# jnsquire/sregex

Hardware: AMD Instinct MI355X
Metric: GB/s input scanned (whole job), gen-data stream resident in HBM (higher is better)
Workload: dtype u8; 1 GPU; configs[1]: /[a-z]+@[a-z]+\.[a-z]+/ Pike first-match + captures; 1 stream x 4.00 GiB gen-data (abccc.. + 'aaabbccb'); bytes_per_gpu=4294967293, streams_per_gpu=1, segment_bytes=16896, fixup_rounds=0, matches=0, engine=scan, lineage_passes=0, world_size=1

## Files before the change

sregex_amd/csrc/sre_hip_scan.hip:

```cpp
#include <hip/hip_runtime.h>
#include <stdlib.h>
#include "sre_hip_scan.h"
#include "sre_hip_streams.h"
#include "sre_hip_tile.h"

#define SRE_HIP_PIKE_COUNT 2
#define EV_DONE 1
#define EV_POP  2
#define RC_DECLINED (-5)
#define RC_ERROR    (-1)


__global__ void
sre_k_gen_data(uint8_t *__restrict__ dst, uint64_t n, uint64_t body, const uint8_t *__restrict__ tail)
{
    const uint64_t stride = (uint64_t) gridDim.x * blockDim.x * 16;
    for (uint64_t base = ((uint64_t) blockIdx.x * blockDim.x + threadIdx.x) * 16; base < n;
         base += stride)
    {
        uint8_t  v[16];
        unsigned ph = (unsigned) (base % 5);
#pragma unroll
        for (int k = 0; k < 16; k++) {
            uint64_t i = base + k;
// ... 130 lines not shown
{
    if (c == '\n') return 1u;
    if (T.word_restart && ((c - '0') < 10u || ((c | 32u) - 'a') < 26u || c == '_')) return 3u;
    return 2u;
}

__device__ inline uint32_t
restart_variant(const sre_scan_tables_t &T, const uint8_t *data, int64_t sp)
{
    return restart_variant_of(T, data[sp - 1]);
}

enum : uint32_t {
    F_HAS_EV = 1u, F_LM_VALID = 2u, F_FINISHED = 4u, F_ERROR = 8u, F_UNRESOLVED = 16u, F_SKIP_NEXT = 32u,
    F_IN_PENDING = 64u, F_SP_DIRTY = 128u,
    F_SHADOW = 256u,
    F_PEND_LAZY = 512u,
    F_NO_EOF = 2048u,
    F_LZ_GROUP = 1024u
};

struct Walk {
    const sre_scan_tables_t *T;
    const uint8_t           *data;
    const uint16_t          *tr2;
    int64_t                  n;
    uint32_t st;
    uint32_t fl;
    __device__ inline bool f(uint32_t b) const { return (fl & b) != 0; }
    __device__ inline void set(uint32_t b, bool v) { fl = v ? (fl | b) : (fl & ~b); }
    uint8_t  ev_kind;
    uint32_t ev_state, ev_sym;
    int64_t  ev_pos, ev_sp;
    int64_t  ev_apos;
    uint32_t ev_astate;
    int64_t  cur_sp;
    int64_t  warm_lo;
    int64_t  anchor_pos;
    uint32_t anchor_state;
    uint32_t lm_state, lm_sym;
    int64_t  lm_pos, lm_sp, lm_apos;
    uint32_t lm_astate;
    int64_t  count;
    int64_t  term_pos;

    __device__ void complete_match()
    {
        count++;
        fl |= F_LM_VALID;
        lm_state = ev_state;
        lm_sym = ev_sym;
        lm_pos = ev_pos;
        lm_sp = ev_sp;
        lm_apos = ev_apos;
        lm_astate = ev_astate;
        fl &= ~F_HAS_EV;
    }
};

template <int MODE>
__device__ void slow_run(Walk &w, int64_t p, int64_t p_to, bool warm, uint32_t warm_seed)
{
    const sre_scan_tables_t &T = *w.T;
    const uint32_t           nsym = T.ncls + 1;
    int64_t  win_at = -1;
    uint64_t win_bytes = 0;
    auto byte_at = [&](int64_t q) -> uint32_t {
        const int64_t a = q & ~(int64_t) 7;
        if (a != win_at) {
            win_at = a;
            if (a + 8 <= w.n && ((reinterpret_cast<uintptr_t>(w.data) + (uint64_t) a) & 7u) == 0) {
                win_bytes = *reinterpret_cast<const uint64_t *>(w.data + a);
            } else {
                win_bytes = 0;
                for (int64_t k = 0; k < 8 && a + k < w.n; k++) win_bytes |= (uint64_t) w.data[a + k] << (8 * k);
            }
        }
        return (uint32_t) (win_bytes >> (8 * (q & 7))) & 0xffu;
    };

    if (MODE == SRE_HIP_PIKE_COUNT && w.f(F_SKIP_NEXT)) {
        w.fl &= ~F_SKIP_NEXT;
        p++;
    }
    while (p < p_to && !w.f(F_FINISHED)) {
        if (p == w.n && ((T.state_flags[w.st] >> 1) & 3) == 2) {
            w.term_pos = p;
            if (MODE == SRE_HIP_PIKE_COUNT) {
                if (w.f(F_HAS_EV)) {
                    w.complete_match();
                    w.fl |= F_ERROR;
                }
            } else if (w.f(F_HAS_EV) || (T.state_flags[w.st] & 1)) {
                w.fl |= F_ERROR;
            }
            w.fl |= F_FINISHED;
            return;
        }
        const uint32_t         sym = p < w.n ? T.cls[byte_at(p)] : T.ncls;
        const uint32_t tr2 = w.tr2[w.st * nsym + sym];
        struct { uint32_t next; uint8_t kind; } tr = {tr2 & 0xffu, (uint8_t) (tr2 >> 8)};
        if (tr.kind) {
            w.fl |= F_HAS_EV;
            w.ev_kind = tr.kind;
            w.ev_state = w.st;
            w.ev_sym = sym;
            w.ev_pos = p;
            w.ev_sp = w.cur_sp;
            if (w.anchor_pos >= 0 && w.anchor_pos <= p && p - w.anchor_pos <= 256
                && (w.cur_sp < 0 || w.anchor_pos > w.cur_sp))
            {
                w.ev_apos = w.anchor_pos;
                w.ev_astate = w.anchor_state;
            } else {
                w.ev_apos = -1;
                w.ev_astate = 0;
            }
            if (MODE != SRE_HIP_PIKE_COUNT && !warm) {
                w.fl |= F_LM_VALID;
                w.lm_state = w.st;
                w.lm_sym = sym;
                w.lm_pos = p;
                w.lm_sp = w.cur_sp;
                w.lm_apos = w.ev_apos;
                w.lm_astate = w.ev_astate;
            }
        }
        w.st = (tr.kind && T.mode == 0 && !warm) ? 0u : tr.next;
        if (w.st != 0) {
            p++;
            continue;
        }

        if (warm) {
            if (MODE == SRE_HIP_PIKE_COUNT) {
                if (w.f(F_HAS_EV)) {
                    const bool    pop = (w.ev_kind == EV_POP || w.ev_kind == SRE_DEV_EV_POP_FULL);
                    const bool    empty = w.ev_kind == EV_POP || w.ev_kind == SRE_DEV_EV_DONE_EMPTY;
                    const int64_t e = pop ? w.ev_pos : w.ev_pos + 1;
                    const int64_t sp = empty ? e + 1 : e;
                    if (e >= w.warm_lo && sp >= 1 && !(empty && e >= w.n)) {
                        w.fl &= ~F_HAS_EV;
                        w.cur_sp = sp;
                        w.st = T.init[restart_variant_of(T, byte_at(sp - 1))];
                        p = sp;
                        if (p > p_to && p_to <= w.n) w.fl |= F_SKIP_NEXT;
                        continue;
                    }
                }
                w.st = p < w.n ? T.init[restart_variant_of(T, byte_at(p))] : warm_seed;
            } else {
                w.st = warm_seed;
            }
            w.fl &= ~F_HAS_EV;
            w.cur_sp = -1;
            p++;
            continue;
        }
        if (MODE != SRE_HIP_PIKE_COUNT) {
            w.term_pos = p;
            w.fl |= F_FINISHED;
            return;
        }
        if (!w.f(F_HAS_EV)) {
            if (p < w.n) w.fl |= F_UNRESOLVED;
            w.term_pos = p;
            w.fl |= F_FINISHED;
            return;
        }
        {
            const bool    pop = (w.ev_kind == EV_POP || w.ev_kind == SRE_DEV_EV_POP_FULL);
            const bool    empty = w.ev_kind == EV_POP || w.ev_kind == SRE_DEV_EV_DONE_EMPTY;
            const int64_t e = pop ? w.ev_pos : w.ev_pos + 1;
            w.complete_match();
            if (empty) {
                if (e >= w.n) {
                    w.term_pos = p;
                    w.fl |= F_FINISHED;
                    return;
                }
                w.cur_sp = e + 1;
            } else {
                w.cur_sp = e;
            }
            w.st = T.init[restart_variant_of(T, byte_at(w.cur_sp - 1))];
            p = w.cur_sp;
            if (p > p_to && p_to <= w.n) w.fl |= F_SKIP_NEXT;
            w.anchor_pos = -1;
        }
    }
}

struct SpanResult {
    int64_t  sp;
    int64_t  last_pos, last_sp;
    uint32_t last_state, last_sym;
    int64_t  pend_pos;
    uint32_t pend_state, pend_sym;
};

__device__ __attribute__((noinline)) SpanResult
resolve_fast_span(const sre_scan_tables_t *Tp, const uint16_t *tr2, const uint8_t *data, int64_t gpos,
                  uint32_t len, uint32_t s0, int64_t sp0, int64_t pend0_pos, uint32_t pend0_state, uint32_t pend0_sym)
{
    const sre_scan_tables_t &T = *Tp;
    SpanResult r;
    uint32_t   st = s0;
    r.sp = sp0;
    r.last_pos = r.last_sp = -1;
    r.last_state = r.last_sym = 0;
    r.pend_pos = pend0_pos;
    r.pend_state = pend0_state;
    r.pend_sym = pend0_sym;
    for (uint32_t b = 0; b < len; b++) {
        const uint32_t         sym = T.cls[data[gpos + b]];
        const uint32_t t2 = tr2[st * (T.ncls + 1) + sym];
        struct { uint32_t next; uint8_t kind; } tr = {t2 & 0xffu, (uint8_t) (t2 >> 8)};
        if (tr.kind && tr.next == 0) {
            const bool pop = tr.kind == SRE_DEV_EV_POP_FULL && gpos + b > 0;
            r.last_pos = gpos + b;
            r.last_state = st;
            r.last_sym = sym;
            r.last_sp = r.sp;
            r.sp = pop ? gpos + b : gpos + b + 1;
            r.pend_pos = -1;
            st = T.init[restart_variant(T, data, r.sp)];
            if (pop) st = tr2[st * (T.ncls + 1) + sym] & 0xffu;
        } else if (tr.kind) {
            r.pend_pos = gpos + b;
            r.pend_state = st;
            r.pend_sym = sym;
            st = tr.next;
        } else if (tr.next == 0 && gpos + b > 0) {
            r.last_pos = r.pend_pos;
            r.last_state = r.pend_state;
            r.last_sym = r.pend_sym;
            r.last_sp = r.sp;
            r.sp = gpos + b;
            st = T.init[restart_variant(T, data, r.sp)];
            const uint32_t t3 = tr2[st * (T.ncls + 1) + sym];
            r.pend_pos = -1;
            if ((t3 >> 8) && (t3 & 0xffu) == 0) {
                r.last_pos = gpos + b;
                r.last_state = st;
                r.last_sym = sym;
                r.last_sp = r.sp;
                r.sp = gpos + b + 1;
                st = T.init[restart_variant(T, data, r.sp)];
            } else {
                if (t3 >> 8) {
                    r.pend_pos = gpos + b;
                    r.pend_state = st;
                    r.pend_sym = sym;
                }
                st = t3 & 0xffu;
            }
        } else {
            st = tr.next;
        }
    }
    return r;
}

template <int H>
__device__ inline uint32_t
add_w0_w(uint32_t a, uint32_t b)
{
    uint32_t r;
    if (H == 0) asm("v_add_u32_sdwa %0, %1, %2 dst_sel:DWORD dst_unused:UNUSED_PAD src0_sel:WORD_0 src1_sel:WORD_0" : "=v"(r) : "v"(a), "v"(b));
    if (H == 1) asm("v_add_u32_sdwa %0, %1, %2 dst_sel:DWORD dst_unused:UNUSED_PAD src0_sel:WORD_0 src1_sel:WORD_1" : "=v"(r) : "v"(a), "v"(b));
    if (H == 2) asm("v_add_u32_sdwa %0, %1, %2 dst_sel:DWORD dst_unused:UNUSED_PAD src0_sel:WORD_0 src1_sel:DWORD" : "=v"(r) : "v"(a), "v"(b));
    return r;
}

__device__ inline uint32_t
add_b3(uint32_t a, uint32_t b)
{
    uint32_t r;
    asm("v_add_u32_sdwa %0, %1, %2 dst_sel:DWORD dst_unused:UNUSED_PAD src0_sel:DWORD src1_sel:BYTE_3" : "=v"(r) : "v"(a), "v"(b));
    return r;
}

template <int K>
__device__ inline uint32_t
byte_x4(uint32_t v, uint32_t sh)
{
    uint32_t r;
    if (K == 0) asm("v_lshlrev_b32_sdwa %0, %1, %2 dst_sel:DWORD dst_unused:UNUSED_PAD src0_sel:DWORD src1_sel:BYTE_0" : "=v"(r) : "v"(sh), "v"(v));
    if (K == 1) asm("v_lshlrev_b32_sdwa %0, %1, %2 dst_sel:DWORD dst_unused:UNUSED_PAD src0_sel:DWORD src1_sel:BYTE_1" : "=v"(r) : "v"(sh), "v"(v));
    if (K == 2) asm("v_lshlrev_b32_sdwa %0, %1, %2 dst_sel:DWORD dst_unused:UNUSED_PAD src0_sel:DWORD src1_sel:BYTE_2" : "=v"(r) : "v"(sh), "v"(v));
    if (K == 3) asm("v_lshlrev_b32_sdwa %0, %1, %2 dst_sel:DWORD dst_unused:UNUSED_PAD src0_sel:DWORD src1_sel:BYTE_3" : "=v"(r) : "v"(sh), "v"(v));
    return r;
}

#ifdef SRE_NO_TAIL_PRIO
#define SRE_TAIL_PRIO() ((void) 0)
#else
#define SRE_TAIL_PRIO() __builtin_amdgcn_s_setprio(3)
#endif

#ifndef SRE_SCAN_PREFETCH
#define SRE_SCAN_PREFETCH 1
#endif
#ifndef SRE_FIRST_BLOCKS
#define SRE_FIRST_BLOCKS 4
#endif
#ifndef SRE_COUNT_BLOCKS
#define SRE_COUNT_BLOCKS 3
#endif

template <int MODE, int BITS, bool WIDE, bool GROW>
__global__ __launch_bounds__(SRE_SCAN_BLOCK, MODE == SRE_HIP_PIKE_COUNT ? SRE_COUNT_BLOCKS : SRE_FIRST_BLOCKS) void
sre_k_scan(const sre_scan_tables_t *__restrict__ tabp, sre_scan_geom_t G,
           sre_seg_summary_t *__restrict__ sum, const sre_stream_status_t *__restrict__ st_lo,
           const uint8_t *__restrict__ entry)
{
    constexpr int      TILE = SRE_SCAN_ROUND;
    constexpr int      WARM = SRE_SCAN_LINE;
    constexpr int      STRIDE = 8 / BITS;
    constexpr uint32_t ROWRAW = TILE / STRIDE * (WIDE ? 2 : 1);
    constexpr uint32_t ROWB = 2 * ROWRAW + 16;
    constexpr int      GIDX = 16 / STRIDE;
    typedef const __attribute__((address_space(3))) uint32_t *lds_u32_t;
    extern __shared__ __attribute__((aligned(16))) uint8_t lds[];
    __shared__ uint16_t clsx[BITS == 8 ? 1 : 8 / BITS][256];
    __shared__ sre_scan_tables_t Ts;

    const uint32_t tid = threadIdx.x;
    const uint32_t nst = tabp->nstates, nrows = tabp->fast_rows, nsh = tabp->nshadow;
    uint32_t *fast = reinterpret_cast<uint32_t *>(lds);
    uint8_t  *clsl = lds + nrows * SRE_FAST_ROW_BYTES;
    uint8_t  *trl = clsl + 256;
    const uint32_t tr_bytes = (nst * (tabp->ncls + 1) * 2u + 15u) & ~15u;
    uint8_t  *sfl = trl + tr_bytes;
    uint8_t  *tile = lds + (((size_t) (sfl - lds) + nst + 15u) & ~(size_t) 15u);
    RowDesc  *rows = reinterpret_cast<RowDesc *>(tile + SRE_SCAN_BLOCK * ROWB);
    (void) nrows;
    if (tid == 0) {
        Ts = *tabp;
        Ts.cls = clsl;
        Ts.state_flags = sfl;
    }
    constexpr uint32_t LDS_SLOW = 1u << 16;
    constexpr uint32_t LDS_CNT_SHIFT = 24;
    constexpr uint32_t LDS_FRESH = 1u << 17;
    const uint32_t fast_lds = (uint32_t) (uintptr_t) (__attribute__((address_space(3))) uint8_t *) lds;
    const uint32_t trap_lds = fast_lds + nst * SRE_FAST_ROW_BYTES;
    const uint32_t shadow_lds = trap_lds + SRE_FAST_ROW_BYTES;
    auto to_lds = [fast_lds, trap_lds](uint32_t g) -> uint32_t {
        if (g & SRE_FAST_SLOW) return trap_lds | LDS_SLOW;
        return (fast_lds + (g & ~(SRE_FAST_ROW_BYTES - 1)))
               | (((g >> SRE_FAST_CNT_SHIFT) & SRE_FAST_CNT_MASK) << LDS_CNT_SHIFT)
               | ((MODE == SRE_HIP_PIKE_COUNT && (g & SRE_FAST_EVT)) ? (128u << LDS_CNT_SHIFT) : 0u)
               | ((MODE == SRE_HIP_PIKE_COUNT && (g & SRE_FAST_NEXT_FRESH)) ? LDS_FRESH : 0u);
    };
    for (uint32_t i = tid; i < nst * 64; i += SRE_SCAN_BLOCK) {
        uint4 e = reinterpret_cast<const uint4 *>(tabp->fast)[i];
        e.x = to_lds(e.x);
        e.y = to_lds(e.y);
        e.z = to_lds(e.z);
        e.w = to_lds(e.w);
        reinterpret_cast<uint4 *>(fast)[i] = e;
    }
    fast[nst * 256 + tid] = trap_lds | LDS_SLOW;
    for (uint32_t q = 0; q < nsh; q++) {
        const uint32_t s = tabp->shadow_state[q], addr = shadow_lds + q * SRE_FAST_ROW_BYTES;
        const uint32_t gl = tabp->fast[s * 256 + tid];
        fast[(nst + 1 + q) * 256 + tid] = (gl & SRE_FAST_STABLE) ? addr : to_lds(gl);
    }
    for (uint32_t i = tid; i < nst * (tabp->ncls + 1); i += SRE_SCAN_BLOCK) {
        reinterpret_cast<uint16_t *>(trl)[i] = tabp->trans2[i];
    }
    for (uint32_t i = tid; i < tabp->nstates; i += SRE_SCAN_BLOCK) sfl[i] = tabp->state_flags[i];
    clsl[tid] = tabp->cls[tid];
    if (BITS != 8) {
#pragma unroll
        for (int u = 0; u < 8 / BITS; u++) clsx[u][tid] = (uint16_t) ((uint32_t) tabp->cls[tid] << (BITS * u + (WIDE ? 2 : 0)));
    }
    __syncthreads();
    const sre_scan_tables_t &T = Ts;

    const uint64_t g = (uint64_t) blockIdx.x * SRE_SCAN_BLOCK + tid;
    bool           active = g < G.nsegs;
    uint32_t       sidx = 0;
    uint64_t       k = 0;
    int64_t        lo_s = -2;
    if (active) {
        uint32_t a = 0, b = G.nstreams;
        while (b - a > 1) {
            uint32_t m = (a + b) >> 1;
            if (geom_first(G, m) <= g) a = m; else b = m;
        }
        sidx = a;
        k = g - geom_first(G, a);
        if (st_lo != nullptr) {
            lo_s = st_lo[sidx].done ? -1 : st_lo[sidx].first_bad;
            if (lo_s < 0 || (int64_t) k < lo_s) active = false;
        }
    }

    Walk w;
    w.T = &T;
    w.tr2 = reinterpret_cast<const uint16_t *>(trl);
    w.data = nullptr;
    w.n = 0;
    w.st = 0;
    w.ev_kind = 0;
    w.ev_state = w.ev_sym = 0;
    w.ev_pos = w.ev_sp = -1;
    w.ev_apos = -1;
    w.ev_astate = 0;
    w.cur_sp = -1;
    w.warm_lo = 0;
    w.anchor_pos = -1;
    w.anchor_state = 0;
    w.lm_state = w.lm_sym = 0;
    w.lm_pos = w.lm_sp = w.lm_apos = -1;
    w.lm_astate = 0;
    w.count = 0;
    w.term_pos = -1;
    w.fl = 0;

    int64_t  seg_a = 0, seg_b = 0;
    uint32_t s_in = 0, seed = 0;
    int64_t  in_pe_pos = -1;
    uint32_t in_pe_state = 0, in_pe_sym = 0;
    bool     last_seg = false, warm = false;
    RowDesc mine;
    mine.addr = 0;
    mine.lo = 0;
    mine.hi16 = -1;
    if (active) {
        w.data = geom_ptr(G, sidx);
        w.n = (int64_t) geom_len(G, sidx);
        seg_a = (int64_t) k * G.seg_bytes;
        seg_b = seg_a + G.seg_bytes;
        const uint64_t nseg = geom_first(G, sidx + 1) - geom_first(G, sidx);
        last_seg = (k + 1 == nseg);
        if (seg_b > w.n) seg_b = w.n;
        if (last_seg && G.sentry != nullptr && (G.sentry[sidx] & SRE_SENTRY_NO_EOF)) w.fl |= F_NO_EOF;

        if (k == 0) {
            w.st = G.sentry != nullptr ? SRE_SENTRY_STATE(G.sentry[sidx])
                   : (G.flags & SRE_GEOM_CONTINUES) ? G.entry_state : T.init[G.init_variant];
            w.cur_sp = 0;
        } else if (lo_s >= 0 && (int64_t) k == lo_s) {
            const sre_seg_summary_t &c = sum[g - 1];
            w.st = c.s_out & ~SRE_STATE_SKIP;
            w.set(F_SKIP_NEXT, MODE == SRE_HIP_PIKE_COUNT && (c.s_out & SRE_STATE_SKIP) != 0);
            w.cur_sp = c.cur_sp;
            if (c.flags & SRE_SUM_PENDING) {
                w.fl |= F_HAS_EV;
                w.ev_state = c.pe_state;
                w.ev_sym = c.pe_sym;
                w.ev_pos = c.pe_pos;
                w.ev_sp = c.pe_sp;
                w.ev_apos = c.pe_apos;
                w.ev_astate = c.pe_astate;
                w.ev_kind = (uint8_t) (w.tr2[c.pe_state * (T.ncls + 1) + c.pe_sym] >> 8);
                if (MODE == SRE_HIP_PIKE_COUNT) {
                    w.fl |= F_IN_PENDING;
                    in_pe_pos = c.pe_pos;
                    in_pe_state = c.pe_state;
                    in_pe_sym = c.pe_sym;
                }
            }
        } else if (entry != nullptr && entry[g] != 0xffu) {
            w.st = entry[g];
            if (MODE == SRE_HIP_PIKE_COUNT && lo_s > 0 && (T.state_flags[w.st] & 1)) {
                const sre_seg_summary_t &c = sum[geom_first(G, sidx) + lo_s - 1];
                if (c.flags & SRE_SUM_PENDING) {
                    w.fl |= F_HAS_EV | F_IN_PENDING;
                    w.ev_state = c.pe_state;
                    w.ev_sym = c.pe_sym;
                    w.ev_pos = c.pe_pos;
                    w.ev_sp = c.pe_sp;
                    w.ev_apos = -1;
                    w.ev_astate = 0;
                    w.ev_kind = (uint8_t) (w.tr2[c.pe_state * (T.ncls + 1) + c.pe_sym] >> 8);
                    in_pe_pos = c.pe_pos;
                    in_pe_state = c.pe_state;
                    in_pe_sym = c.pe_sym;
                }
            }
        } else {
            warm = true;
            seed = T.init[0];
            if (lo_s > 0) {
                const sre_seg_summary_t &c = sum[geom_first(G, sidx) + lo_s - 1];
                const uint32_t           cs = c.s_out & ~SRE_STATE_SKIP;
                if (cs != 0) {
                    if (!(MODE == SRE_HIP_PIKE_COUNT && (T.state_flags[cs] & 1))) {
                        seed = cs;
                    } else if (c.flags & SRE_SUM_PENDING) {
                        seed = cs;
                        w.fl |= F_HAS_EV;
                        w.ev_state = c.pe_state;
                        w.ev_sym = c.pe_sym;
                        w.ev_pos = c.pe_pos;
                        w.ev_sp = c.pe_sp;
                        w.ev_apos = -1;
                        w.ev_astate = 0;
                        w.ev_kind = (uint8_t) (w.tr2[c.pe_state * (T.ncls + 1) + c.pe_sym] >> 8);
                    }
                }
            }
            w.st = seed;
        }
        w.warm_lo = seg_a >= (int64_t) WARM ? seg_a - (int64_t) WARM : 0;
        s_in = w.st | (MODE == SRE_HIP_PIKE_COUNT && w.f(F_SKIP_NEXT) ? SRE_STATE_SKIP : 0u);
        mine.addr = (uint64_t) reinterpret_cast<uintptr_t>(w.data) + (uint64_t) (seg_a - WARM);
        mine.lo = warm ? (seg_a >= WARM ? 0 : (int32_t) (WARM - seg_a)) : WARM;
        mine.hi16 = (int32_t) (WARM + (seg_b - seg_a)) - 16;
    }
    rows[tid] = mine;

    int64_t  fcA_pos = -1, fcB_pos = -1, fc_sp0 = -1;
    uint32_t fcA_len = 0, fcA_s0 = 0, fcB_len = 0, fcB_s0 = 0;
    int64_t  lz_pos = -1;
    uint32_t lz_s0 = 0;
    auto note_span = [&](int64_t pos, uint32_t len, uint32_t s0, uint32_t cnt, bool warm_round) {
        w.fl &= ~F_HAS_EV;
        if (warm_round) return;
        if (w.f(F_SP_DIRTY)) {
            fcA_pos = fcB_pos;
            fcA_len = fcB_len;
            fcA_s0 = fcB_s0;
        } else {
            fc_sp0 = w.cur_sp;
            fcA_pos = -1;
        }
        fcB_pos = pos;
        fcB_len = len;
        fcB_s0 = s0;
        if (w.f(F_PEND_LAZY)) {
            fcB_pos = lz_pos;
            fcB_len = len + (w.f(F_LZ_GROUP) ? 16u : (uint32_t) TILE);
            fcB_s0 = lz_s0;
        }
        w.fl |= F_SP_DIRTY;
        w.count += cnt;
    };
    constexpr bool any_fresh = GROW;
    auto fast_span_done = [&](int64_t pos, uint32_t len, uint32_t s0, uint32_t sum, bool fresh1, bool warm_round) {
        if (!any_fresh) {
            if (sum) note_span(pos, len, s0, sum, warm_round);
            return;
        }
        if (sum == 0) {
            w.fl &= ~F_PEND_LAZY;
            return;
        }
        if (sum & 127u) note_span(pos, len, s0, sum & 127u, warm_round);
        else if (sum) w.fl &= ~F_HAS_EV;
        if (fresh1) {
            w.fl |= F_PEND_LAZY;
            w.set(F_LZ_GROUP, len == 16u);
            lz_pos = pos;
            lz_s0 = s0;
        } else {
            w.fl &= ~F_PEND_LAZY;
        }
    };
    auto settle = [&]() {
        if (MODE != SRE_HIP_PIKE_COUNT || !(w.fl & (F_SP_DIRTY | F_PEND_LAZY))) return;
        if (w.f(F_SP_DIRTY)) {
            int64_t sp0 = fc_sp0;
            if (fcA_pos >= 0) sp0 = resolve_fast_span(&T, w.tr2, w.data, fcA_pos, fcA_len, fcA_s0, -1, -1, 0, 0).sp;
            const SpanResult r = resolve_fast_span(&T, w.tr2, w.data, fcB_pos, fcB_len, fcB_s0, sp0, w.ev_pos, w.ev_state, w.ev_sym);
            if (r.last_pos >= 0) {
                w.fl |= F_LM_VALID;
                w.lm_pos = r.last_pos;
                w.lm_state = r.last_state;
                w.lm_sym = r.last_sym;
                w.lm_sp = r.last_sp;
                const bool anchored = r.last_sp < fcB_pos && r.last_pos - fcB_pos <= 256 && fcB_pos >= seg_a;
                w.lm_apos = anchored ? fcB_pos : (int64_t) -1;
                w.lm_astate = anchored ? fcB_s0 : 0u;
            }
            w.cur_sp = r.sp;
            w.fl &= ~F_SP_DIRTY;
        }
        if (w.f(F_PEND_LAZY)) {
            const SpanResult r = resolve_fast_span(&T, w.tr2, w.data, lz_pos, w.f(F_LZ_GROUP) ? 16u : (uint32_t) TILE, lz_s0,
                                                   -1, -1, 0, 0);
            w.fl &= ~F_PEND_LAZY;
            if (r.pend_pos >= 0) {
                w.fl |= F_HAS_EV;
                w.ev_pos = r.pend_pos;
                w.ev_state = r.pend_state;
                w.ev_sym = r.pend_sym;
                w.ev_kind = (uint8_t) (w.tr2[r.pend_state * (T.ncls + 1) + r.pend_sym] >> 8);
                w.ev_sp = w.cur_sp;
                const bool anchored = w.cur_sp < lz_pos && lz_pos >= seg_a;
                w.ev_apos = anchored ? lz_pos : (int64_t) -1;
                w.ev_astate = anchored ? lz_s0 : 0u;
            }
        }
    };

    constexpr uint32_t SU_UNSET = 0xffffffffu;
    uint32_t           su = SU_UNSET, run_off = 0;
    static_assert(SRE_SCAN_MAX_SHADOWS == 2, "two shadow rows");
    const uint32_t sh_st0 = nsh > 0 ? tabp->shadow_state[0] : 0xffffu, sh_st1 = nsh > 1 ? tabp->shadow_state[1] : 0xffffu;
    const uint32_t sh_ad0 = shadow_lds, sh_ad1 = shadow_lds + SRE_FAST_ROW_BYTES;
    const uint32_t     two = 2;
    (void) two;

    const uint32_t nrounds = WARM / TILE + G.seg_bytes / TILE;
    const uint32_t lag = (tid >> 5) & 1u;
    constexpr uint32_t DIST = SRE_SCAN_PREFETCH;
    __syncthreads();
    auto round = [&](const uint32_t s, uint4 (&regs)[4]) __attribute__((always_inline)) {
        __builtin_amdgcn_fence(__ATOMIC_ACQ_REL, "wavefront");
        __builtin_amdgcn_wave_barrier();
        tile_store<BITS, WIDE>(regs, tile, clsx, tid, s);
        __builtin_amdgcn_fence(__ATOMIC_ACQ_REL, "wavefront");
        __builtin_amdgcn_wave_barrier();
        if (s + DIST <= nrounds) tile_fetch(regs, rows, tid, s + DIST);

        if (s < lag || s - lag >= nrounds) return;
        const uint32_t r = s - lag;
        const bool     warm_round = (r < WARM / TILE);
        if (!active || w.f(F_FINISHED) || (warm_round && !warm)) return;
        const int64_t base = seg_a - WARM + (int64_t) r * TILE;
        if (base >= seg_b || base < 0) return;
        w.anchor_pos = warm_round ? -1 : base;
        w.anchor_state = w.st;

        constexpr int ROWW = (ROWRAW + 3) / 4;
        uint32_t      roww[ROWW < 4 ? 4 : ROWW];
        {
            const uint8_t *src = tile + tid * ROWB + (r & 1u) * ROWRAW;
            if (ROWW >= 4) {
#pragma unroll
                for (int x = 0; x < ROWW / 4; x++) {
                    const uint4 v = *reinterpret_cast<const uint4 *>(src + 16 * x);
                    roww[4 * x] = v.x; roww[4 * x + 1] = v.y; roww[4 * x + 2] = v.z; roww[4 * x + 3] = v.w;
                }
            } else if (ROWW == 2) {
                const uint2 v = *reinterpret_cast<const uint2 *>(src);
                roww[0] = v.x; roww[1] = v.y;
            } else {
                roww[0] = *reinterpret_cast<const uint32_t *>(src);
            }
        }
        if (base + TILE <= seg_b && !(MODE == SRE_HIP_PIKE_COUNT && w.f(F_SKIP_NEXT))) {
            uint32_t t = fast_lds + w.st * SRE_FAST_ROW_BYTES, cnt = 0;
            if (MODE != SRE_HIP_PIKE_COUNT && !warm_round) {
                const uint32_t sha = w.st == sh_st0 ? sh_ad0 : w.st == sh_st1 ? sh_ad1 : 0u;
                if (!w.f(F_SHADOW)) {
                    if (sha) {
                        w.fl |= F_SHADOW;
                        run_off = (uint32_t) (base - seg_a);
                    } else if (su == SU_UNSET) {
                        su = (uint32_t) (base - seg_a);
                    }
                }
                if (w.f(F_SHADOW)) t = sha;
            }
#pragma unroll
            for (int j = 0; j < TILE * BITS / 8; j++) {
                uint32_t a;
                if (WIDE) {
                    a = (j & 1) ? add_w0_w<1>(t, roww[j >> 1]) : add_w0_w<0>(t, roww[j >> 1]);
                } else {
                    const uint32_t wj = roww[j >> 2];
                    const uint32_t ix = (j & 3) == 0 ? byte_x4<0>(wj, two) : (j & 3) == 1 ? byte_x4<1>(wj, two)
                                      : (j & 3) == 2 ? byte_x4<2>(wj, two) : byte_x4<3>(wj, two);
                    a = add_w0_w<2>(t, ix);
                }
                t = *(lds_u32_t) (uintptr_t) a;
                if (MODE == SRE_HIP_PIKE_COUNT) cnt = add_b3(cnt, t);
            }
            if (!(t & LDS_SLOW)) {
                const uint32_t ridx = ((t & 0xffffu) - fast_lds) / SRE_FAST_ROW_BYTES;
                if (MODE == SRE_HIP_PIKE_COUNT) fast_span_done(base, TILE, w.st, cnt, (t & LDS_FRESH) != 0, warm_round);
                w.st = MODE == SRE_HIP_PIKE_COUNT ? ridx : ridx <= nst ? ridx : ridx == nst + 1 ? sh_st0 : sh_st1;
                if (MODE != SRE_HIP_PIKE_COUNT && w.f(F_SHADOW) && ridx <= nst) {
                    w.fl &= ~F_SHADOW;
                    if (su == SU_UNSET) su = (uint32_t) (base - seg_a);
                }
                if (r + 1 == WARM / TILE) {
                    s_in = w.st | (MODE == SRE_HIP_PIKE_COUNT && w.f(F_SKIP_NEXT) ? SRE_STATE_SKIP : 0u);
                    settle();
                    w.cur_sp = -1;
                    if (w.f(F_HAS_EV)) w.ev_sp = -1;
                    if (w.st == 0) w.fl |= F_FINISHED;
                    if (MODE == SRE_HIP_PIKE_COUNT) {
                        w.set(F_IN_PENDING, w.f(F_HAS_EV));
                        in_pe_pos = w.ev_pos;
                        in_pe_state = w.ev_state;
                        in_pe_sym = w.ev_sym;
                    }
                }
                return;
            }
        }
        if (MODE != SRE_HIP_PIKE_COUNT && !warm_round) {
            w.fl &= ~F_SHADOW;
            if (su == SU_UNSET) su = (uint32_t) (base - seg_a);
        }
#pragma unroll 1
        for (uint32_t q = 0; q < TILE / 16; q++) {
            const int64_t gp = base + q * 16;
            if (gp >= seg_b || w.f(F_FINISHED)) break;
            const int64_t g_end = gp + 16 <= seg_b ? gp + 16 : seg_b;
            bool          exact = (g_end != gp + 16) || (MODE == SRE_HIP_PIKE_COUNT && w.f(F_SKIP_NEXT));
            uint32_t      t = fast_lds + w.st * SRE_FAST_ROW_BYTES, cnt = 0;
            if (!exact) {
                constexpr int GW = GIDX * (WIDE ? 2 : 1) / 4;
                uint32_t      gw[GW];
                const uint32_t *gsrc = reinterpret_cast<const uint32_t *>(tile + tid * ROWB + (r & 1u) * ROWRAW) + q * GW;
#pragma unroll
                for (int x = 0; x < GW; x++) gw[x] = gsrc[x];
#pragma unroll
                for (int j = 0; j < GIDX; j++) {
                    const uint32_t ix = WIDE ? (gw[j >> 1] >> ((j & 1) * 16)) & 0xffffu
                                             : ((gw[j >> 2] >> ((j & 3) * 8)) & 0xffu) << 2;
                    t = *(lds_u32_t) (uintptr_t) ((t & 0xffffu) + ix);
                    if (MODE == SRE_HIP_PIKE_COUNT) cnt += t >> LDS_CNT_SHIFT;
                }
                exact = (t & LDS_SLOW) != 0;
            }
            if (exact) {
                settle();
                slow_run<MODE>(w, gp, g_end, warm_round, seed);
            } else {
                const uint32_t st1 = ((t & 0xffffu) - fast_lds) / SRE_FAST_ROW_BYTES;
                if (MODE == SRE_HIP_PIKE_COUNT) fast_span_done(gp, 16, w.st, cnt, (t & LDS_FRESH) != 0, warm_round);
                w.st = st1;
            }
        }
        if (r + 1 == WARM / TILE) {
            s_in = w.st | (MODE == SRE_HIP_PIKE_COUNT && w.f(F_SKIP_NEXT) ? SRE_STATE_SKIP : 0u);
            settle();
            w.cur_sp = -1;
            if (w.f(F_HAS_EV)) w.ev_sp = -1;
            if (w.st == 0) w.fl |= F_FINISHED;
            if (MODE == SRE_HIP_PIKE_COUNT) {
                w.set(F_IN_PENDING, w.f(F_HAS_EV));
                in_pe_pos = w.ev_pos;
                in_pe_state = w.ev_state;
                in_pe_sym = w.ev_sym;
            }
        }
    
    };
    uint4 regs[4];
    tile_fetch(regs, rows, tid, 0);
    if (DIST == 1) {
        for (uint32_t s = 0; s <= nrounds; s++) round(s, regs);
    } else {
        uint4 regs2[4];
        if (nrounds >= 1) tile_fetch(regs2, rows, tid, 1);
        for (uint32_t s = 0; s <= nrounds; s += 2) {
            round(s, regs);
            if (s + 1 <= nrounds) round(s + 1, regs2);
        }
    }

    if (!active) return;

    if (last_seg && !w.f(F_FINISHED) && !(G.flags & SRE_GEOM_NO_EOF) && !w.f(F_NO_EOF)) {
        settle();
        w.anchor_pos = -1;
        slow_run<MODE>(w, w.n, w.n + 1, false, 0);
    }
    settle();

    sre_seg_summary_t out;
    {
        const uint32_t seg_len = (uint32_t) (seg_b - seg_a);
        if (MODE == SRE_HIP_PIKE_COUNT || (w.f(F_FINISHED) && su == SU_UNSET)) su = 0;
        out.stable_until = su == SU_UNSET ? seg_len : su;
        out.stable_from = (MODE != SRE_HIP_PIKE_COUNT && w.f(F_SHADOW)) ? run_off : seg_len;
    }
    out.s_in = w.f(F_UNRESOLVED) ? 0xffffffffu : s_in;
    out.s_out = w.st | (MODE == SRE_HIP_PIKE_COUNT && w.f(F_SKIP_NEXT) ? SRE_STATE_SKIP : 0u);
    out.flags = 0;
    out.pad = 0;
    out.count = w.count;
    out.term_pos = w.term_pos;
    out.cur_sp = w.cur_sp;
    if (w.f(F_FINISHED) && w.term_pos >= 0) out.flags |= SRE_SUM_TERM;
    if (w.f(F_ERROR)) out.flags |= SRE_SUM_ERROR;
    if (w.f(F_HAS_EV)) out.flags |= SRE_SUM_PENDING;
    if (w.f(F_LM_VALID)) out.flags |= SRE_SUM_LASTEV;
    if (MODE == SRE_HIP_PIKE_COUNT && w.f(F_IN_PENDING)) out.flags |= SRE_SUM_IN_PENDING;
    if (MODE != SRE_HIP_PIKE_COUNT && out.stable_until == G.seg_bytes && !last_seg) out.flags |= SRE_SUM_STABLE;
    out.in_pe_pos = in_pe_pos;
    out.in_pe_state = in_pe_state;
    out.in_pe_sym = in_pe_sym;
    out.pe_state = w.ev_state;
    out.pe_sym = w.ev_sym;
    out.pe_pos = w.ev_pos;
    out.pe_sp = w.ev_sp;
    out.lm_state = w.lm_state;
    out.lm_sym = w.lm_sym;
    out.lm_pos = w.lm_pos;
    out.lm_sp = w.lm_sp;
    out.lm_apos = w.lm_apos;
    out.lm_astate = w.lm_astate;
    out.pe_apos = w.ev_apos;
    out.pe_astate = w.ev_astate;
    sum[g] = out;
    if (MODE != SRE_HIP_PIKE_COUNT && G.digest != nullptr) {
        sre_seg_digest_t dg;
        dg.s_in = out.s_in;
        dg.s_out = out.s_out;
        dg.bits = ((out.flags & SRE_SUM_TERM) ? 2u : 0u) | ((out.flags & SRE_SUM_LASTEV) ? 4u : 0u) | (out.cur_sp >= 0 ? 8u : 0u)
                  | ((out.flags & SRE_SUM_STABLE) ? 0u : 16u);
        dg.count = (uint32_t) out.count;
        G.digest[g] = dg;
    }
}


#define SRE_FN_CHUNK 256u

template <int BITS>
__global__ __launch_bounds__(256) void
sre_k_seg_functions(const sre_scan_tables_t *__restrict__ tabp, sre_scan_geom_t G,
                    const sre_stream_status_t *__restrict__ status, uint8_t *__restrict__ fn)
{
    constexpr int STRIDE = 8 / BITS;
    constexpr int GIDX = 16 / STRIDE;
    typedef const __attribute__((address_space(3))) uint32_t *lds_u32_t;
    extern __shared__ __attribute__((aligned(16))) uint8_t lds[];
    __shared__ uint16_t clsx[BITS == 8 ? 1 : 8 / BITS][256];
    const uint32_t tid = threadIdx.x, nst = tabp->nstates, nsym = tabp->ncls + 1;
    uint32_t *fast = reinterpret_cast<uint32_t *>(lds);
    uint8_t  *clsl = lds + (nst + 1) * SRE_FAST_ROW_BYTES;
    uint16_t *tr2 = reinterpret_cast<uint16_t *>(clsl + 256);
    constexpr uint32_t LDS_SLOW = 1u << 16;
    const uint32_t fast_lds = (uint32_t) (uintptr_t) (__attribute__((address_space(3))) uint8_t *) lds;
    const uint32_t trap_lds = fast_lds + nst * SRE_FAST_ROW_BYTES;
    for (uint32_t i = tid; i < nst * 256; i += 256) {
        const uint32_t gl = tabp->fast[i];
        fast[i] = (gl & SRE_FAST_SLOW) ? (trap_lds | LDS_SLOW) : fast_lds + (gl & ~(SRE_FAST_ROW_BYTES - 1));
    }
    fast[nst * 256 + tid] = trap_lds | LDS_SLOW;
    clsl[tid] = tabp->cls[tid];
    for (uint32_t i = tid; i < nst * nsym; i += 256) tr2[i] = tabp->trans2[i];
    if (BITS != 8) {
#pragma unroll
        for (int u = 0; u < 8 / BITS; u++) clsx[u][tid] = (uint16_t) ((uint32_t) tabp->cls[tid] << (BITS * u + 2));
    }
    __syncthreads();

    const uint32_t lane = tid & 63u;
    const uint64_t g = (uint64_t) blockIdx.x * 4 + (tid >> 6);
    if (g >= G.nsegs) return;
    const uint32_t s = stream_of(G, g);
    const uint64_t k = g - geom_first(G, s);
    if (status[s].done || (int64_t) k < status[s].first_bad) return;
    if (lane >= nst) {
        fn[g * 64 + lane] = 0;
        return;
    }
    const uint8_t *data = geom_ptr(G, s);
    const int64_t  n = (int64_t) geom_len(G, s);
    int64_t        p = (int64_t) k * G.seg_bytes, seg_b = p + G.seg_bytes;
    if (seg_b > n) seg_b = n;
    uint32_t cur = lane;
    const bool count_mode = tabp->mode == SRE_HIP_PIKE_COUNT;
    auto exact = [&](int64_t from, int64_t to) {
        if (!count_mode) {
            for (int64_t q = from; q < to; q++) cur = tr2[cur * nsym + clsl[data[q]]] & 0xffu;
            return;
        }
        int64_t  pend = -1;
        uint32_t pkind = 0, guard = 0;
        for (int64_t q = from; q < to; q++) {
            const uint32_t sym = clsl[data[q]];
            const uint32_t t2 = tr2[cur * nsym + sym];
            if (t2 >> 8) {
                pend = q;
                pkind = t2 >> 8;
            }
            cur = t2 & 0xffu;
            if (cur != 0) continue;
            int64_t sp = q + 1;
            if (pend >= 0) {
                const bool    pop = pkind == EV_POP || pkind == SRE_DEV_EV_POP_FULL;
                const bool    empty = pkind == EV_POP || pkind == SRE_DEV_EV_DONE_EMPTY;
                const int64_t e = pop ? pend : pend + 1;
                sp = empty ? e + 1 : e;
            } else if (++guard < 2) {
                sp = q;
            }
            if (pend >= 0) guard = 0;
            if (sp < 1) sp = 1;
            if (sp > n) sp = n;
            cur = tabp->init[restart_variant_of(*tabp, data[sp - 1])];
            pend = -1;
            q = sp - 1;
        }
    };
    for (; p + 16 <= seg_b; p += 16) {
        const sre_u32x4 v = *reinterpret_cast<const __attribute__((address_space(1))) sre_u32x4_unaligned *>(
            reinterpret_cast<uintptr_t>(data + p));
        const uint32_t words[4] = {v.x, v.y, v.z, v.w};
        uint32_t       t = fast_lds + cur * SRE_FAST_ROW_BYTES;
#pragma unroll
        for (int j = 0; j < GIDX; j++) {
            uint32_t ix = 0;
#pragma unroll
            for (int u = 0; u < STRIDE; u++) {
                const int      b = j * STRIDE + u;
                const uint32_t c = (words[b >> 2] >> ((b & 3) * 8)) & 0xffu;
                ix |= BITS == 8 ? c << 2 : (uint32_t) clsx[u][c];
            }
            t = *(lds_u32_t) (uintptr_t) ((t & 0xffffu) + ix);
        }
        if (t & LDS_SLOW) exact(p, p + 16);
        else cur = ((t & 0xffffu) - fast_lds) / SRE_FAST_ROW_BYTES;
    }
    exact(p, seg_b);
    fn[g * 64 + lane] = (uint8_t) cur;
}

__global__ __launch_bounds__(64) void
sre_k_fn_chunks(uint64_t nsegs, const uint8_t *__restrict__ fn, uint8_t *__restrict__ comp)
{
    const uint64_t c = blockIdx.x;
    uint32_t       v = threadIdx.x;
    const uint64_t g0 = c * SRE_FN_CHUNK, g1 = g0 + SRE_FN_CHUNK <= nsegs ? g0 + SRE_FN_CHUNK : nsegs;
    for (uint64_t g = g0; g < g1; g++) v = fn[g * 64 + (v & 63u)];
    comp[c * 64 + threadIdx.x] = (uint8_t) v;
}

__global__ void
sre_k_fn_resolve(sre_scan_geom_t G, const sre_seg_summary_t *__restrict__ sum,
                 const sre_stream_status_t *__restrict__ status, const uint8_t *__restrict__ fn,
                 const uint8_t *__restrict__ comp, uint8_t *__restrict__ entry, uint8_t *__restrict__ chunk_entry)
{
    const uint32_t s = blockIdx.x * blockDim.x + threadIdx.x;
    if (s >= G.nstreams || status[s].done || status[s].first_bad < 1) return;
    const uint64_t first = geom_first(G, s), g_hi = geom_first(G, s + 1);
    uint64_t       g = first + (uint64_t) status[s].first_bad;
    uint32_t       v = sum[g - 1].s_out & 63u;
    while (g < g_hi) {
        if (g % SRE_FN_CHUNK == 0 && g + SRE_FN_CHUNK <= g_hi) {
            chunk_entry[g / SRE_FN_CHUNK] = (uint8_t) v;
            v = comp[(g / SRE_FN_CHUNK) * 64 + v];
            g += SRE_FN_CHUNK;
        } else {
            entry[g] = (uint8_t) v;
            v = fn[g * 64 + v];
            g++;
        }
    }
}

__global__ void
sre_k_fn_fill(uint64_t nsegs, const uint8_t *__restrict__ fn, const uint8_t *__restrict__ chunk_entry,
              uint8_t *__restrict__ entry)
{
    const uint64_t c = (uint64_t) blockIdx.x * blockDim.x + threadIdx.x;
    if (c * SRE_FN_CHUNK >= nsegs || chunk_entry[c] == 0xffu) return;
    uint32_t v = chunk_entry[c];
    for (uint64_t g = c * SRE_FN_CHUNK; g < (c + 1) * SRE_FN_CHUNK && g < nsegs; g++) {
        entry[g] = (uint8_t) v;
        v = fn[g * 64 + (v & 63u)];
    }
}


struct VerifyAcc {
    unsigned long long bad, end;
    unsigned long long count, evseg, spseg;
    unsigned long long unst;
    unsigned long long unst_end;
};

__global__ __launch_bounds__(256) void
sre_k_verify_a(sre_scan_geom_t G, const sre_seg_summary_t *__restrict__ sum, VerifyAcc *__restrict__ acc,
               int mode)
{
    SRE_TAIL_PRIO();
    const uint64_t g = (uint64_t) blockIdx.x * blockDim.x + threadIdx.x;
    const bool     valid = g < G.nsegs;
    const uint32_t s = stream_of(G, valid ? g : G.nsegs - 1);
    unsigned long long kb = ~0ull, ke = ~0ull;
    if (valid) {
        const uint64_t k = g - geom_first(G, s);
        const uint32_t s_in = sum[g].s_in;
        bool           bad = s_in == 0xffffffffu;
        if (k > 0) {
            const sre_seg_summary_t &p = sum[g - 1], &c = sum[g];
            if (s_in != p.s_out) bad = true;
            if (mode == SRE_HIP_PIKE_COUNT) {
                const bool pp = (p.flags & SRE_SUM_PENDING) != 0, cp = (c.flags & SRE_SUM_IN_PENDING) != 0;
                if (pp != cp) bad = true;
                if (pp && cp && (p.pe_pos != c.in_pe_pos || p.pe_state != c.in_pe_state || p.pe_sym != c.in_pe_sym)) {
                    bad = true;
                }
            }
        }
        if (bad) kb = k;
        if (sum[g].flags & SRE_SUM_TERM) ke = k;
    }
    const uint32_t s0 = (uint32_t) __builtin_amdgcn_readfirstlane((int) s);
    if (__builtin_amdgcn_ballot_w64(s != s0) == 0) {
        for (int d = 32; d >= 1; d >>= 1) {
            const unsigned long long ob = __shfl_xor(kb, d, 64), oe = __shfl_xor(ke, d, 64);
            kb = ob < kb ? ob : kb;
            ke = oe < ke ? oe : ke;
        }
        if ((threadIdx.x & 63u) != 0) kb = ke = ~0ull;
    }
    if (kb != ~0ull && kb < __hip_atomic_load(&acc[s].bad, __ATOMIC_RELAXED, __HIP_MEMORY_SCOPE_AGENT)) atomicMin(&acc[s].bad, kb);
    if (ke != ~0ull && ke < __hip_atomic_load(&acc[s].end, __ATOMIC_RELAXED, __HIP_MEMORY_SCOPE_AGENT)) atomicMin(&acc[s].end, ke);
}

#define SRE_VERIFY_SPAN 1024u

__global__ __launch_bounds__(256) void
sre_k_verify_b(sre_scan_geom_t G, const sre_seg_summary_t *__restrict__ sum, VerifyAcc *__restrict__ acc)
{
    SRE_TAIL_PRIO();
    __shared__ unsigned long long sh_count, sh_ev, sh_sp;
    const uint64_t g0 = (uint64_t) blockIdx.x * SRE_VERIFY_SPAN;
    const uint64_t glast = (g0 + SRE_VERIFY_SPAN - 1 < G.nsegs) ? g0 + SRE_VERIFY_SPAN - 1 : G.nsegs - 1;
    const uint32_t s_first = stream_of(G, g0), s_last = stream_of(G, glast);
    const bool     uniform = (s_first == s_last);
    if (threadIdx.x == 0) {
        sh_count = 0;
        sh_ev = 0;
        sh_sp = 0;
    }
    __syncthreads();
    unsigned long long my_count = 0, my_ev = 0, my_sp = 0;
    for (uint32_t it = 0; it < SRE_VERIFY_SPAN / 256; it++) {
        const uint64_t g = g0 + it * 256u + threadIdx.x;
        if (g >= G.nsegs) break;
        const uint32_t s = uniform ? s_first : stream_of(G, g);
        const uint64_t k = g - geom_first(G, s);
        const uint64_t nseg = geom_first(G, s + 1) - geom_first(G, s);
        uint64_t       bad = acc[s].bad, end = acc[s].end;
        if (bad > nseg) bad = nseg;
        if (end > nseg) end = nseg;
        const uint64_t limit = end < bad ? end + 1 : bad;
        if (k < limit) {
            const sre_seg_summary_t &c = sum[g];
            if (uniform) {
                my_count += (unsigned long long) c.count;
                if (c.flags & SRE_SUM_LASTEV) my_ev = (unsigned long long) k + 1;
                if (c.cur_sp >= 0) my_sp = (unsigned long long) k + 1;
            } else {
                if (c.count) atomicAdd(&acc[s].count, (unsigned long long) c.count);
                if (c.flags & SRE_SUM_LASTEV) atomicMax(&acc[s].evseg, (unsigned long long) k + 1);
                if (c.cur_sp >= 0) atomicMax(&acc[s].spseg, (unsigned long long) k + 1);
            }
        }
    }
    if (uniform) {
// ... 1633 lines not shown
```

sregex_amd/csrc/sre_hip_tile.h:

```cpp
#ifndef SRE_HIP_TILE_H
#define SRE_HIP_TILE_H

#include <hip/hip_runtime.h>
#include "sre_hip_scan.h"

namespace {

struct __attribute__((aligned(16))) RowDesc {
    uint64_t addr;
    int32_t  lo;
    int32_t  hi16;
};

typedef uint32_t sre_u32x4 __attribute__((ext_vector_type(4)));
typedef sre_u32x4 __attribute__((aligned(1))) sre_u32x4_unaligned;

__device__ inline void
tile_fetch(uint4 (&regs)[4], const RowDesc *rows, uint32_t tid, uint32_t stage)
{
    const uint32_t wbase = (tid & ~63u) + (stage & 1u) * 32u, lane = tid & 63u;
    const int32_t  line_off = (int32_t) ((stage >> 1) * SRE_SCAN_LINE);
#pragma unroll
    for (uint32_t i = 0; i < 4; i++) {
        const uint32_t piece = i * 64 + lane;
        const uint32_t row = wbase + piece / 8, col = piece % 8;
        const int32_t  off = line_off + (int32_t) (col * 16);
        const uint4    d = *reinterpret_cast<const uint4 *>(&rows[row]);
        sre_u32x4      v = {0, 0, 0, 0};
        if ((off >= (int32_t) d.z) & (off <= (int32_t) d.w)) {
            const uint64_t a = (((uint64_t) d.y << 32) | d.x) + (uint64_t) (int64_t) off;
            v = *reinterpret_cast<const __attribute__((address_space(1))) sre_u32x4_unaligned *>(a);
        }
        regs[i] = make_uint4(v.x, v.y, v.z, v.w);
    }
}

template <int BITS, bool WIDE>
__device__ inline void
tile_store(const uint4 (&regs)[4], uint8_t *tile, const uint16_t (*clsx)[256], uint32_t tid, uint32_t stage)
{
    constexpr int      STRIDE = 8 / BITS;
    constexpr uint32_t HALFB = SRE_SCAN_ROUND / STRIDE * (WIDE ? 2 : 1);
    constexpr uint32_t ROWB = 2 * HALFB + 16;
    constexpr uint32_t PIECEB = HALFB / 4;
    const uint32_t wbase = (tid & ~63u) + (stage & 1u) * 32u, lane = tid & 63u;
#pragma unroll
    for (uint32_t i = 0; i < 4; i++) {
        const uint32_t piece = i * 64 + lane;
        const uint32_t row = wbase + piece / 8, col = piece % 8;
        const uint32_t words[4] = {regs[i].x, regs[i].y, regs[i].z, regs[i].w};
        uint8_t       *dst = tile + row * ROWB + col * PIECEB;
        if (BITS == 8) {
            *reinterpret_cast<uint4 *>(dst) = regs[i];
        } else {
            constexpr int NIDX = 16 / STRIDE;
            constexpr int PERW = WIDE ? 2 : 4;
            uint32_t      out[NIDX / PERW];
#pragma unroll
            for (int k = 0; k < NIDX; k++) {
                uint32_t v = 0;
#pragma unroll
                for (int u = 0; u < STRIDE; u++) {
                    const int      b = k * STRIDE + u;
                    const uint32_t c = (words[b >> 2] >> ((b & 3) * 8)) & 0xffu;
                    v |= (uint32_t) clsx[u][c];
                }
                if (k % PERW) out[k / PERW] |= v << ((k % PERW) * (32 / PERW)); else out[k / PERW] = v;
            }
            constexpr int NW = NIDX / PERW;
            if (PIECEB == 4) *reinterpret_cast<uint32_t *>(dst) = out[0];
            else if (PIECEB == 8) *reinterpret_cast<uint2 *>(dst) = make_uint2(out[0], out[1 % NW]);
            else *reinterpret_cast<uint4 *>(dst) = make_uint4(out[0], out[1 % NW], out[2 % NW], out[3 % NW]);
        }
    }
}

constexpr uint32_t SRE_TILE2_ROWB = SRE_SCAN_ROUND + 16;

__device__ inline void
tile2_fetch(uint4 (&regs)[4], const RowDesc *rows, uint32_t tid, uint32_t stage)
{
    const uint32_t wbase = (tid & ~63u) + (stage & 1u) * 32u, lane = tid & 63u;
    const int32_t  line_off = (int32_t) ((stage >> 1) * SRE_SCAN_LINE);
#pragma unroll
    for (uint32_t i = 0; i < 4; i++) {
        const uint32_t row = wbase + (lane >> 2) + 16u * (i >> 1), col = (lane & 3u) + 4u * (i & 1u);
        const int32_t  off = line_off + (int32_t) (col * 16);
        const uint4    d = *reinterpret_cast<const uint4 *>(&rows[row]);
        sre_u32x4      v = {0, 0, 0, 0};
        if ((off >= (int32_t) d.z) & (off <= (int32_t) d.w)) {
            const uint64_t a = (((uint64_t) d.y << 32) | d.x) + (uint64_t) (int64_t) off;
            v = *reinterpret_cast<const __attribute__((address_space(1))) sre_u32x4_unaligned *>(a);
        }
        regs[i] = make_uint4(v.x, v.y, v.z, v.w);
    }
}

__device__ inline void
tile2_store(const uint4 (&regs)[4], uint4 (&hold)[2], uint8_t *tile, uint32_t tid, uint32_t stage)
{
    const uint32_t wave = tid & ~63u, lane = tid & 63u, h = stage & 1u;
    const uint32_t rnew = wave + h * 32u + (lane >> 2), rold = wave + (1u - h) * 32u + (lane >> 2);
    const uint32_t col = (lane & 3u) * 16u;
    *reinterpret_cast<uint4 *>(tile + rnew * SRE_TILE2_ROWB + col) = regs[0];
    *reinterpret_cast<uint4 *>(tile + (rnew + 16u) * SRE_TILE2_ROWB + col) = regs[2];
    *reinterpret_cast<uint4 *>(tile + rold * SRE_TILE2_ROWB + col) = hold[0];
    *reinterpret_cast<uint4 *>(tile + (rold + 16u) * SRE_TILE2_ROWB + col) = hold[1];
    hold[0] = regs[1];
    hold[1] = regs[3];
}

}

#endif
```

Before: 5442 GB/s.

## Add wave-uniform fast path for tile fetch when segment rows are contiguous

Before the scan loop, each wave works out whether the 32 rows of each half-wave map to contiguous, equally spaced segments, plus the range of 128-byte lines every row can read. For stages inside that range, the fetch uses one scalar base address and a precomputed per-lane offset with no per-lane bounds checks. This replaces the per-piece LDS row-descriptor load and range test in tile_fetch. It adds some shuffles and readlanes at setup, and a branch on every fetch, while the old path stays as the fallback.

```diff
diff --git a/sregex_amd/csrc/sre_hip_scan.hip b/sregex_amd/csrc/sre_hip_scan.hip
--- a/sregex_amd/csrc/sre_hip_scan.hip
+++ b/sregex_amd/csrc/sre_hip_scan.hip
@@ -456,6 +456,9 @@
 #ifndef SRE_SCAN_PREFETCH
 #define SRE_SCAN_PREFETCH 1
 #endif
+#ifndef SRE_SCAN_UNIFORM_FETCH
+#define SRE_SCAN_UNIFORM_FETCH 1
+#endif
 #ifndef SRE_FIRST_BLOCKS
 #define SRE_FIRST_BLOCKS 4
 #endif
@@ -580,10 +583,7 @@
     int64_t  in_pe_pos = -1;
     uint32_t in_pe_state = 0, in_pe_sym = 0;
     bool     last_seg = false, warm = false;
-    RowDesc mine;
-    mine.addr = 0;
-    mine.lo = 0;
-    mine.hi16 = -1;
+    RowDesc mine = tile_row_none();
     if (active) {
         w.data = geom_ptr(G, sidx);
         w.n = (int64_t) geom_len(G, sidx);
@@ -663,9 +663,7 @@
         }
         w.warm_lo = seg_a >= (int64_t) WARM ? seg_a - (int64_t) WARM : 0;
         s_in = w.st | (MODE == SRE_HIP_PIKE_COUNT && w.f(F_SKIP_NEXT) ? SRE_STATE_SKIP : 0u);
-        mine.addr = (uint64_t) reinterpret_cast<uintptr_t>(w.data) + (uint64_t) (seg_a - WARM);
-        mine.lo = warm ? (seg_a >= WARM ? 0 : (int32_t) (WARM - seg_a)) : WARM;
-        mine.hi16 = (int32_t) (WARM + (seg_b - seg_a)) - 16;
+        mine = tile_row_desc((uint64_t) reinterpret_cast<uintptr_t>(w.data), seg_a, seg_b, warm);
     }
     rows[tid] = mine;
 
@@ -765,13 +763,25 @@
     const uint32_t lag = (tid >> 5) & 1u;
     constexpr uint32_t DIST = SRE_SCAN_PREFETCH;
     __syncthreads();
+    const uint32_t lane_off = tile_uniform_lane_off(tid & 63u, G.seg_bytes);
+    const uint32_t wgeom = SRE_SCAN_UNIFORM_FETCH ? tile_wave_geom(mine, tid, G.seg_bytes) : 0u;
+    auto fetch = [&](const uint32_t s, uint4 (&regs)[4]) __attribute__((always_inline)) {
+        if (SRE_SCAN_UNIFORM_FETCH) {
+            const HalfGeom h = tile_stage_geom(wgeom, s);
+            if (tile_line_uniform(h, s >> 1)) {
+                tile_fetch_uniform(regs, h, s >> 1, G.seg_bytes, lane_off);
+                return;
+            }
+        }
+        tile_fetch(regs, rows, tid, s);
+    };
     auto round = [&](const uint32_t s, uint4 (&regs)[4]) __attribute__((always_inline)) {
         __builtin_amdgcn_fence(__ATOMIC_ACQ_REL, "wavefront");
         __builtin_amdgcn_wave_barrier();
         tile_store<BITS, WIDE>(regs, tile, clsx, tid, s);
         __builtin_amdgcn_fence(__ATOMIC_ACQ_REL, "wavefront");
         __builtin_amdgcn_wave_barrier();
-        if (s + DIST <= nrounds) tile_fetch(regs, rows, tid, s + DIST);
+        if (s + DIST <= nrounds) fetch(s + DIST, regs);
 
         if (s < lag || s - lag >= nrounds) return;
         const uint32_t r = s - lag;
@@ -902,12 +912,12 @@
     
     };
     uint4 regs[4];
-    tile_fetch(regs, rows, tid, 0);
+    fetch(0, regs);
     if (DIST == 1) {
         for (uint32_t s = 0; s <= nrounds; s++) round(s, regs);
     } else {
         uint4 regs2[4];
-        if (nrounds >= 1) tile_fetch(regs2, rows, tid, 1);
+        if (nrounds >= 1) fetch(1, regs2);
         for (uint32_t s = 0; s <= nrounds; s += 2) {
             round(s, regs);
             if (s + 1 <= nrounds) round(s + 1, regs2);
diff --git a/sregex_amd/csrc/sre_hip_tile.h b/sregex_amd/csrc/sre_hip_tile.h
--- a/sregex_amd/csrc/sre_hip_tile.h
+++ b/sregex_amd/csrc/sre_hip_tile.h
@@ -3,14 +3,9 @@
 
 #include <hip/hip_runtime.h>
 #include "sre_hip_scan.h"
+#include "sre_tile_geom.h"
 
 namespace {
-
-struct __attribute__((aligned(16))) RowDesc {
-    uint64_t addr;
-    int32_t  lo;
-    int32_t  hi16;
-};
 
 typedef uint32_t sre_u32x4 __attribute__((ext_vector_type(4)));
 typedef sre_u32x4 __attribute__((aligned(1))) sre_u32x4_unaligned;
@@ -33,6 +28,53 @@
         }
         regs[i] = make_uint4(v.x, v.y, v.z, v.w);
     }
+}
+
+__device__ inline void
+tile_fetch_uniform(uint4 (&regs)[4], const HalfGeom &h, uint32_t line, uint32_t seg_bytes, uint32_t lane_off)
+{
+    static_assert(SRE_GEOM_LINE == SRE_SCAN_LINE, "one staging granule");
+    asm volatile("" : "+v"(lane_off));
+    uint64_t b = tile_uniform_base(h, line, 0, seg_bytes);
+#pragma unroll
+    for (uint32_t i = 0; i < 4; i++, b += 8u * seg_bytes) {
+        const __attribute__((address_space(1))) uint8_t *p = reinterpret_cast<const __attribute__((address_space(1))) uint8_t *>(b);
+        const sre_u32x4 v = *reinterpret_cast<const __attribute__((address_space(1))) sre_u32x4_unaligned *>(p + lane_off);
+        regs[i] = make_uint4(v.x, v.y, v.z, v.w);
+    }
+    asm volatile("");
+}
+
+__device__ inline uint32_t
+tile_wave_geom(const RowDesc &mine, uint32_t tid, uint32_t seg_bytes)
+{
+    const uint32_t lane = tid & 63u, j = lane & 31u, half = lane & 32u;
+    const uint32_t alo = (uint32_t) mine.addr, ahi = (uint32_t) (mine.addr >> 32);
+    int32_t        lo = mine.lo, hi = mine.hi16;
+#pragma unroll
+    for (int m = 1; m < 32; m <<= 1) {
+        const int32_t lo2 = __shfl_xor(lo, m), hi2 = __shfl_xor(hi, m);
+        lo = lo2 > lo ? lo2 : lo;
+        hi = hi2 < hi ? hi2 : hi;
+    }
+    const uint32_t f0lo = (uint32_t) __builtin_amdgcn_readlane((int) alo, 0), f0hi = (uint32_t) __builtin_amdgcn_readlane((int) ahi, 0);
+    const uint32_t f1lo = (uint32_t) __builtin_amdgcn_readlane((int) alo, 32), f1hi = (uint32_t) __builtin_amdgcn_readlane((int) ahi, 32);
+    const uint64_t first = half ? ((uint64_t) f1hi << 32) | f1lo : ((uint64_t) f0hi << 32) | f0lo;
+    const uint64_t ok = __ballot(tile_row_contiguous(mine.addr, first, j, seg_bytes));
+    const uint32_t okh = half ? (uint32_t) (ok >> 32) : (uint32_t) ok;
+    const HalfGeom h = tile_half_geom(first, okh == 0xffffffffu, lo, hi, seg_bytes);
+    return j == 0 ? (uint32_t) h.first : j == 1 ? (uint32_t) (h.first >> 32) : j == 2 ? h.line_beg : h.line_end;
+}
+
+__device__ inline HalfGeom
+tile_stage_geom(uint32_t gv, uint32_t stage)
+{
+    const int at = (int) ((stage & 1u) * 32u);
+    HalfGeom  h;
+    h.first = ((uint64_t) (uint32_t) __builtin_amdgcn_readlane((int) gv, at + 1) << 32) | (uint32_t) __builtin_amdgcn_readlane((int) gv, at);
+    h.line_beg = (uint32_t) __builtin_amdgcn_readlane((int) gv, at + 2);
+    h.line_end = (uint32_t) __builtin_amdgcn_readlane((int) gv, at + 3);
+    return h;
 }
 
 template <int BITS, bool WIDE>
diff --git a/sregex_amd/csrc/sre_tile_geom.h b/sregex_amd/csrc/sre_tile_geom.h
--- /dev/null
+++ b/sregex_amd/csrc/sre_tile_geom.h
@@ -0,0 +1,117 @@
+#ifndef SRE_TILE_GEOM_H
+#define SRE_TILE_GEOM_H
+
+#include <stdint.h>
+
+#if defined(__HIPCC__)
+#define SRE_GEOM_FN __host__ __device__ inline
+#else
+#define SRE_GEOM_FN inline
+#endif
+
+namespace {
+
+struct __attribute__((aligned(16))) RowDesc {
+    uint64_t addr;
+    int32_t  lo;
+    int32_t  hi16;
+};
+
+constexpr uint32_t SRE_GEOM_LINE = 128;
+constexpr uint32_t SRE_GEOM_HALF = 32;
+
+SRE_GEOM_FN RowDesc
+tile_row_none()
+{
+    RowDesc d;
+    d.addr = 0;
+    d.lo = 0;
+    d.hi16 = -1;
+    return d;
+}
+
+SRE_GEOM_FN RowDesc
+tile_row_desc(uint64_t data, int64_t seg_a, int64_t seg_b, bool warm)
+{
+    constexpr int64_t W = (int64_t) SRE_GEOM_LINE;
+    RowDesc           d;
+    d.addr = data + (uint64_t) (seg_a - W);
+    d.lo = warm ? (seg_a >= W ? 0 : (int32_t) (W - seg_a)) : (int32_t) W;
+    d.hi16 = (int32_t) (W + (seg_b - seg_a)) - 16;
+    return d;
+}
+
+SRE_GEOM_FN uint32_t
+tile_piece_row(uint32_t lane, uint32_t i)
+{
+    return (i * 64 + lane) / 8;
+}
+SRE_GEOM_FN int32_t
+tile_piece_off(uint32_t lane, uint32_t stage)
+{
+    return (int32_t) ((stage >> 1) * SRE_GEOM_LINE + (lane % 8) * 16);
+}
+SRE_GEOM_FN bool
+tile_piece_readable(const RowDesc &d, int32_t off)
+{
+    return (off >= d.lo) & (off <= d.hi16);
+}
+
+struct HalfGeom {
+    uint64_t first;
+    uint32_t line_beg;
+    uint32_t line_end;
+};
+
+SRE_GEOM_FN bool
+tile_geom_fits32(uint32_t seg_bytes)
+{
+    return seg_bytes < (1u << 29);
+}
+SRE_GEOM_FN bool
+tile_row_contiguous(uint64_t addr, uint64_t first, uint32_t j, uint32_t seg_bytes)
+{
+    return addr == first + (uint64_t) j * seg_bytes;
+}
+SRE_GEOM_FN HalfGeom
+tile_half_geom(uint64_t first, bool contiguous, int32_t lo_max, int32_t hi16_min, uint32_t seg_bytes)
+{
+    HalfGeom h;
+    h.first = first;
+    h.line_beg = lo_max <= 0 ? 0u : ((uint32_t) lo_max + SRE_GEOM_LINE - 1) / SRE_GEOM_LINE;
+    h.line_end = hi16_min >= 112 ? ((uint32_t) hi16_min - 112u) / SRE_GEOM_LINE + 1u : 0u;
+    if (!contiguous || !tile_geom_fits32(seg_bytes) || h.line_end < h.line_beg) h.line_end = h.line_beg;
+    return h;
+}
+SRE_GEOM_FN bool
+tile_line_uniform(const HalfGeom &h, uint32_t line)
+{
+    return line - h.line_beg < h.line_end - h.line_beg;
+}
+SRE_GEOM_FN uint32_t
+tile_uniform_lane_off(uint32_t lane, uint32_t seg_bytes)
+{
+    return (lane / 8) * seg_bytes + 16 * (lane % 8);
+}
+SRE_GEOM_FN uint64_t
+tile_uniform_base(const HalfGeom &h, uint32_t line, uint32_t i, uint32_t seg_bytes)
+{
+    return h.first + (uint64_t) line * SRE_GEOM_LINE + (uint64_t) i * (8 * seg_bytes);
+}
+
+SRE_GEOM_FN HalfGeom
+tile_half_geom_rows(const RowDesc *rows, uint32_t seg_bytes)
+{
+    bool    contiguous = true;
+    int32_t lo_max = rows[0].lo, hi16_min = rows[0].hi16;
+    for (uint32_t j = 0; j < SRE_GEOM_HALF; j++) {
+        contiguous = contiguous & tile_row_contiguous(rows[j].addr, rows[0].addr, j, seg_bytes);
+        lo_max = rows[j].lo > lo_max ? rows[j].lo : lo_max;
+        hi16_min = rows[j].hi16 < hi16_min ? rows[j].hi16 : hi16_min;
+    }
+    return tile_half_geom(rows[0].addr, contiguous, lo_max, hi16_min, seg_bytes);
+}
+
+}
+
+#endif
```

Measured after the change: 5439 GB/s. No clear change (-0.0%).
